# pimdh/lie-vae

Hardware: AMD Instinct MI355X
Metric: SO(3) samples/sec (exp+WignerD+action, l_max=10) (higher is better)
Workload: dtype f32

## Files before the change

### lie-vae_amd/csrc/action.hip

```cpp
#include <algorithm>
#include <cmath>
#include <cstdlib>
#include <array>
#include <atomic>
#include <vector>

#include "action_kernels.h"

namespace lv {
LV_EXTERN_LAUNCHERS(0) LV_EXTERN_LAUNCHERS(1) LV_EXTERN_LAUNCHERS(2) LV_EXTERN_LAUNCHERS(3)
LV_EXTERN_LAUNCHERS(4) LV_EXTERN_LAUNCHERS(5) LV_EXTERN_LAUNCHERS(6) LV_EXTERN_LAUNCHERS(7)
LV_EXTERN_LAUNCHERS(8) LV_EXTERN_LAUNCHERS(9) LV_EXTERN_LAUNCHERS(10) LV_EXTERN_LAUNCHERS(11)
LV_EXTERN_LAUNCHERS(12) LV_EXTERN_LAUNCHERS(13) LV_EXTERN_LAUNCHERS(14) LV_EXTERN_LAUNCHERS(15)
LV_EXTERN_LAUNCHERS(16) LV_EXTERN_LAUNCHERS(17) LV_EXTERN_LAUNCHERS(18) LV_EXTERN_LAUNCHERS(19)
LV_EXTERN_LAUNCHERS(20)
LV_EXTERN_BWD(0) LV_EXTERN_BWD(1) LV_EXTERN_BWD(2) LV_EXTERN_BWD(3) LV_EXTERN_BWD(4)
LV_EXTERN_BWD(5) LV_EXTERN_BWD(6) LV_EXTERN_BWD(7) LV_EXTERN_BWD(8) LV_EXTERN_BWD(9)
LV_EXTERN_BWD(10) LV_EXTERN_BWD(11) LV_EXTERN_BWD(12) LV_EXTERN_BWD(13) LV_EXTERN_BWD(14)
LV_EXTERN_BWD(15) LV_EXTERN_BWD(16) LV_EXTERN_BWD(17) LV_EXTERN_BWD(18) LV_EXTERN_BWD(19)
LV_EXTERN_BWD(20)

#ifndef LV_REDUCE_COLS
#define LV_REDUCE_COLS 16
#endif
constexpr int kBwdReduceCols = LV_REDUCE_COLS;
constexpr int kBwdReduceStreams = 64 / kBwdReduceCols;
__global__ __launch_bounds__(64 * kBwdReduceWaves) void action_bwd_reduce_kernel(
    const float* ws_F, float* gF, int64_t MC, int nslab) {
  __shared__ float part[kBwdReduceWaves][64];
  const int lane = threadIdx.x & 63, w = threadIdx.x >> 6;
  const int k = lane / kBwdReduceCols, col = lane - k * kBwdReduceCols;
  const int64_t e = (int64_t)blockIdx.x * kBwdReduceCols + col;
  const int per = (nslab + kBwdReduceWaves - 1) / kBwdReduceWaves;
  const int b0 = min(nslab, w * per), b1 = min(nslab, b0 + per);
  float sum = 0.f;
  if (e < MC) {
    int b = b0 + k;
    constexpr int S = kBwdReduceStreams;
    for (; b + 7 * S < b1; b += 8 * S) {
      float v[8];
#pragma unroll
      for (int u = 0; u < 8; ++u) v[u] = ws_F[(int64_t)(b + u * S) * MC + e];
#pragma unroll
      for (int u = 0; u < 8; ++u) sum += v[u];
    }
    for (; b < b1; b += S) sum += ws_F[(int64_t)b * MC + e];
  }
  part[w][lane] = sum;
  __syncthreads();
  if (threadIdx.x < kBwdReduceCols && e < MC) {
    float r = 0.f;
    for (int ww = 0; ww < kBwdReduceWaves; ++ww) {
      float rw = part[ww][col];
#pragma unroll
      for (int kk = 1; kk < kBwdReduceStreams; ++kk) rw += part[ww][kk * kBwdReduceCols + col];
      r += rw;
    }
    gF[e] = r;
  }
}

template <int COLS>
__global__ __launch_bounds__(1024) void action_bwd_reduce2_kernel(const float* ws_F, float* gF, int64_t MC,
                                                                  int nslab) {
  constexpr int S = 1024 / COLS;
  __shared__ float part[S][COLS];
  const int col = (int)threadIdx.x % COLS, k = (int)threadIdx.x / COLS;
  const int64_t e = (int64_t)blockIdx.x * COLS + col;
  float sum = 0.f;
  if (e < MC) {
    int b = k;
    for (; b + 7 * S < nslab; b += 8 * S) {
      float v[8];
#pragma unroll
      for (int u = 0; u < 8; ++u) v[u] = ws_F[(int64_t)(b + u * S) * MC + e];
#pragma unroll
      for (int u = 0; u < 8; ++u) sum += v[u];
    }
    for (; b < nslab; b += S) sum += ws_F[(int64_t)b * MC + e];
  }
  part[k][col] = sum;
#pragma unroll
  for (int h = S / 2; h >= 1; h >>= 1) {
    __syncthreads();
    if (k < h) part[k][col] += part[k + h][col];
  }
  if (k == 0 && e < MC) gF[e] = part[0][col];
}

__global__ __launch_bounds__(1024) void action_bwd_reduce3_kernel(const float* ws_F, float* gF, int64_t MC,
                                                                  int nslab, unsigned long long* stamps) {
  typedef float f4 __attribute__((ext_vector_type(4)));
  unsigned long long* rst = stamps ? stamps + kStampBlocks * 16 * 8 + 2 * (int64_t)blockIdx.x : nullptr;
  if (rst && threadIdx.x == 0) rst[0] = __builtin_amdgcn_s_memrealtime();
  __shared__ f4 part[256][4];
  const int q = (int)threadIdx.x & 3, bs = (int)threadIdx.x >> 2;
  const f4* base = reinterpret_cast<const f4*>(ws_F + (int64_t)blockIdx.x * nslab * kSlabChunk) + q;
  f4 acc = {0.f, 0.f, 0.f, 0.f};
  int b = bs;
  for (; b + 3 * 256 < nslab; b += 4 * 256) {
    f4 v[4];
#pragma unroll
    for (int u = 0; u < 4; ++u) v[u] = base[(int64_t)(b + u * 256) * 4];
#pragma unroll
    for (int u = 0; u < 4; ++u) acc += v[u];
  }
  {
    f4 v[3];
#pragma unroll
    for (int u = 0; u < 3; ++u) v[u] = b + u * 256 < nslab ? base[(int64_t)(b + u * 256) * 4] : f4{0.f, 0.f, 0.f, 0.f};
#pragma unroll
    for (int u = 0; u < 3; ++u)
      if (b + u * 256 < nslab) acc += v[u];
  }
  part[bs][q] = acc;
#pragma unroll
  for (int h = 128; h >= 1; h >>= 1) {
    __syncthreads();
    if (bs < h) part[bs][q] += part[bs + h][q];
  }
  if (bs == 0) {
    const f4 r = part[0][q];
#pragma unroll
    for (int k = 0; k < 4; ++k) {
      const int64_t e = (int64_t)blockIdx.x * kSlabChunk + 4 * q + k;
      if (e < MC) gF[e] = r[k];
    }
    if (rst) rst[1] = __builtin_amdgcn_s_memrealtime();
  }
}

__global__ __launch_bounds__(1024) void action_bwd_reduce4_kernel(const float* ws_F, float* gF, int64_t MC,
                                                                  int nslab) {
  typedef float f4 __attribute__((ext_vector_type(4)));
  __shared__ f4 part[16][4];
  const int q = (int)threadIdx.x & 3, bs = (int)threadIdx.x >> 2;
  const f4* base = reinterpret_cast<const f4*>(ws_F + (int64_t)blockIdx.x * nslab * kSlabChunk) + q;
  f4 acc = {0.f, 0.f, 0.f, 0.f};
  int b = bs;
  for (; b + 3 * 256 < nslab; b += 4 * 256) {
    f4 v[4];
#pragma unroll
    for (int u = 0; u < 4; ++u) v[u] = base[(int64_t)(b + u * 256) * 4];
#pragma unroll
    for (int u = 0; u < 4; ++u) acc += v[u];
  }
  {
    f4 v[3];
#pragma unroll
    for (int u = 0; u < 3; ++u) v[u] = b + u * 256 < nslab ? base[(int64_t)(b + u * 256) * 4] : f4{0.f, 0.f, 0.f, 0.f};
#pragma unroll
    for (int u = 0; u < 3; ++u)
      if (b + u * 256 < nslab) acc += v[u];
  }
#pragma unroll
  for (int m = 4; m <= 32; m <<= 1) {
#pragma unroll
    for (int k = 0; k < 4; ++k) acc[k] += __shfl_xor(acc[k], m, 64);
  }
  const int w = (int)threadIdx.x >> 6, lane = (int)threadIdx.x & 63;
  if (lane < 4) part[w][lane] = acc;
  __syncthreads();
  if (threadIdx.x < 4) {
    f4 r = part[0][q];
#pragma unroll
    for (int ww = 1; ww < 16; ++ww) r += part[ww][q];
#pragma unroll
    for (int k = 0; k < 4; ++k) {
      const int64_t e = (int64_t)blockIdx.x * kSlabChunk + 4 * q + k;
      if (e < MC) gF[e] = r[k];
    }
  }
}

constexpr int kR5Loads = 12;
__device__ __forceinline__ void reduce5_chunk(const float* ws_F, float* gF, int64_t MC, int nslab, int chunk) {
// ... 25 lines not shown
#pragma unroll
    for (int ww = 1; ww < 4; ++ww) r += part[ww][q];
#pragma unroll
    for (int k = 0; k < 4; ++k) {
      const int64_t e = (int64_t)chunk * kSlabChunk + 4 * q + k;
      if (e < MC) gF[e] = r[k];
    }
  }
}
__global__ __launch_bounds__(256) void action_bwd_reduce5_kernel(const float* ws_F, float* gF, int64_t MC, int nslab) {
  reduce5_chunk(ws_F, gF, MC, nslab, (int)blockIdx.x);
}

__global__ __launch_bounds__(256) void action_bwd_reduce5_vjp_kernel(const float* ws_F, float* gF, int64_t MC,
                                                                     int nslab, int nvjp, const float* mu,
                                                                     const float* v, const float* gang,
                                                                     float* gmu, float* gv, int64_t n) {
  if ((int)blockIdx.x < nvjp) {
    const int64_t i = (int64_t)blockIdx.x * 256 + threadIdx.x;
    if (i < n) {
      float av[3], g[3], m[9], gm[9], o[3];
#pragma unroll
      for (int k = 0; k < 3; ++k) { av[k] = v[i * 3 + k]; g[k] = gang[i * 3 + k]; }
      if (mu) {
#pragma unroll
        for (int k = 0; k < 9; ++k) m[k] = mu[i * 9 + k];
      }
      exp_eazyz_vjp_sample_wide(av, mu != nullptr, m, g, gm, o);
      if (mu) {
#pragma unroll
        for (int k = 0; k < 9; ++k) gmu[i * 9 + k] = gm[k];
      }
#pragma unroll
      for (int k = 0; k < 3; ++k) gv[i * 3 + k] = o[k];
    }
    return;
  }
  reduce5_chunk(ws_F, gF, MC, nslab, (int)blockIdx.x - nvjp);
}

namespace {

template <int... Ls>
constexpr std::array<int, sizeof...(Ls)> nnz_table(std::integer_sequence<int, Ls...>) {
  return {j_nnz<Ls>()...};
}
constexpr auto kNnz = nnz_table(std::make_integer_sequence<int, LV_MAX_DEGREE + 1>{});

inline double degree_cost(int l, bool bwd) {
  const int n = 2 * l + 1;
  const double fwd = 2.0 * kNnz[l] + 6.0 * n + 3.0 * n;
  return bwd ? 2.2 * fwd : fwd;
}

inline int plan_segments(int L, int nseg, double P, bool bwd, int* seg_lo) {
  constexpr int kD = LV_MAX_DEGREE + 1;
  const int D = L + 1;
  nseg = std::max(1, std::min(nseg, std::min(D, kMaxSeg)));
  double pre[kD + 1];
  pre[0] = 0.0;
  for (int l = 0; l < D; ++l) pre[l + 1] = pre[l] + degree_cost(l, bwd);
  const double INF = 1e30;
  double dp[kMaxSeg + 1][kD + 1];
  int arg[kMaxSeg + 1][kD + 1];
  for (int k = 0; k <= nseg; ++k)
    for (int i = 0; i <= D; ++i) { dp[k][i] = INF; arg[k][i] = 0; }
  dp[0][0] = 0.0;
  for (int k = 1; k <= nseg; ++k)
    for (int i = 1; i <= D; ++i)
      for (int p = k - 1; p < i; ++p) {
        const double v = std::max(dp[k - 1][p], pre[i] - pre[p] + P);
        if (v < dp[k][i]) { dp[k][i] = v; arg[k][i] = p; }
      }
  int i = D;
  for (int k = nseg; k >= 1; --k) {
    seg_lo[k] = i;
    i = arg[k][i];
  }
  seg_lo[0] = 0;
  return nseg;
}

constexpr double kDegFixedFwd = 80.0, kDegFixedBwd = 30.0;
inline double degree_cost_sched(int l, bool bwd) {
  return (bwd ? kDegFixedBwd : kDegFixedFwd) + degree_cost(l, bwd);
}
inline void balance_masks(int L, int nseg, bool bwd, unsigned* masks) {
  double load[kMaxSeg];
  for (int k = 0; k < nseg; ++k) { load[k] = 0.0; masks[k] = 0u; }
  for (int l = L; l >= 0; --l) {
    int best = 0;
    for (int k = 1; k < nseg; ++k)
      if (load[k] < load[best]) best = k;
    masks[best] |= 1u << l;
    load[best] += degree_cost_sched(l, bwd);
  }
  for (int k = nseg; k < kMaxSeg; ++k) masks[k] = 0u;
}
inline void contiguous_masks(const int* seg_lo, int nseg, unsigned* masks) {
  for (int k = 0; k < kMaxSeg; ++k) {
    masks[k] = 0u;
    if (k < nseg)
      for (int l = seg_lo[k]; l < seg_lo[k + 1]; ++l) masks[k] |= 1u << l;
  }
}

inline int choose_nseg(int64_t n, int Sw, int L, double P, bool bwd) {
  const int64_t waves = (n + Sw - 1) / Sw;
  const int64_t target = 2732;
  int nseg = (int)std::min<int64_t>(kMaxSeg, std::max<int64_t>(1, (target + waves - 1) / waves));
  double total = 0.0;
  for (int l = 0; l <= L; ++l) total += degree_cost(l, bwd);
  const int cap = std::max(1, (int)(total / (2.0 * P)));
  return std::min(nseg, std::min(cap, L + 1));
}

constexpr double kPrologueFwd = 200.0;
constexpr double kPrologueFused = 250.0;

constexpr size_t kTileMaxLds = 80 * 1024;
constexpr double kTileSegCostFew = 300.0;
constexpr double kTileSegCostMid = 260.0;
constexpr double kTileSegCostLarge = 560.0;
constexpr int64_t kTileFewGroupsPerCU = 4, kTileMidGroupsPerCU = 16;
constexpr double kTilePrologue = 60.0;
constexpr int64_t kWriteThroughMaxBytes = 32ll << 20;

#ifdef LV_AB_KNOBS
int env_int(const char* name, int dflt) {
  const char* v = std::getenv(name);
  return v && *v ? std::atoi(v) : dflt;
}
#define LV_KNOB(name, dflt) env_int(name, dflt)
constexpr size_t kStampBytes = sizeof(unsigned long long) * ((size_t)kStampDegBase + kStampDegBlocks * 16 * 24);
unsigned long long* ab_stamps() {
  static unsigned long long* p = nullptr;
  static bool tried = false;
  if (!tried) {
    tried = true;
    if (env_int("LV_STAMPS", 0) && hipMalloc(&p, kStampBytes) == hipSuccess) (void)hipMemset(p, 0, kStampBytes);
  }
  return p;
}
bool env_masks(const char* name, int L, int nseg, unsigned* masks) {
  const char* v = std::getenv(name);
  if (!v || !*v) return false;
  unsigned m[kMaxSeg] = {};
  int k = 0;
  unsigned all = 0;
  for (const char* s = v; *s && k < kMaxSeg;) {
    char* e = nullptr;
    m[k] = (unsigned)std::strtoul(s, &e, 16);
    if (e == s || (m[k] & all) || m[k] == 0) return false;
    all |= m[k++];
    s = (*e == ',' || *e == ':') ? e + 1 : e;
  }
  if (k != nseg || all != (1u << (L + 1)) - 1) return false;
  for (int i = 0; i < kMaxSeg; ++i) masks[i] = i < nseg ? m[i] : 0u;
  return true;
}
#else
#define LV_KNOB(name, dflt) (dflt)
inline unsigned long long* ab_stamps() { return nullptr; }
inline bool env_masks(const char*, int, int, unsigned*) { return false; }
#endif

int device_cus();

bool plan_tile(FwdLaunch& p, int L, int out_bytes, int cus) {
  static const int kEnvTile = LV_KNOB("LV_TILE", 1);
  static const int kEnvWT = LV_KNOB("LV_TILE_WT", -1);
  static const int kEnvTileNseg = LV_KNOB("LV_TILE_NSEG", 0);
  static const int kEnvPrio = LV_KNOB("LV_TILE_PRIO", 2);
  static const int kEnvSw = LV_KNOB("LV_TILE_SW", 0);
  if (!kEnvTile) return false;
  ActionArgs& a = p.a;
  int Sw = 64 / a.C;
  if (a.C == kTileFastC && kEnvSw >= 2 && kEnvSw < Sw) Sw = kEnvSw;
  const int64_t groups = (a.n + Sw - 1) / Sw;
  double total = 0.0;
  for (int l = 0; l <= L; ++l) total += degree_cost(l, false);
  const double target = groups <= kTileFewGroupsPerCU * cus   ? kTileSegCostFew
                        : groups <= kTileMidGroupsPerCU * cus ? kTileSegCostMid
                                                              : kTileSegCostLarge;
  int nseg = std::max(1, std::min(std::min(8, L + 1), (int)std::ceil(total / target)));
  if (kEnvTileNseg > 0) nseg = std::min(std::min(8, L + 1), kEnvTileNseg);
  nseg = std::min(L + 1, std::max(nseg, (3 * Sw + 63) / 64));
  if (3 * Sw > 64 * nseg || nseg > 8) return false;
  plan_segments(L, nseg, kTilePrologue, false, a.seg_lo);
  static const int kEnvContig = LV_KNOB("LV_SEG_CONTIG", 0);
  if (a.C == kTileFastC && env_masks("LV_TILE_MASKS", L, nseg, a.seg_mask)) {
  } else if (a.C == kTileFastC && !kEnvContig) balance_masks(L, nseg, false, a.seg_mask);
  else contiguous_masks(a.seg_lo, nseg, a.seg_mask);
  int fp = 0;
  if (a.C != kTileFastC && L < kTileFGlobalMinL)
    for (int k = 0; k < nseg; ++k) fp = std::max(fp, fseg_rows(a.seg_lo[k], a.seg_lo[k + 1]) * a.C);
  a.fpitch = (fp + 3) & ~3;
  const size_t fl = a.C == kTileFastC ? (out_bytes == 4 ? 0 : (size_t)a.MC) : (size_t)nseg * a.fpitch;
  const size_t trig = (size_t)Sw * (6 * ((L + 1 + 3) & ~3) + 4);
  const size_t lds = (size_t)tile_stage_bytes(Sw, a.MC, out_bytes) + sizeof(float) * (fl + trig);
  if (lds > kTileMaxLds || groups > 0x7fffffff) return false;
  a.Sw = Sw;
  a.write_through = (int64_t)a.n * a.MC * out_bytes <= kWriteThroughMaxBytes ? 1 : 0;
  if (kEnvWT >= 0) a.write_through = kEnvWT;
  a.prio = kEnvPrio;
  static const int kEnvSpread = LV_KNOB("LV_TILE_SPREAD", 0);
  a.task_spread = kEnvSpread;
  static const int kEnvAngOrder = LV_KNOB("LV_TILE_ANG_ORDER", 0);
  a.ang_order = kEnvAngOrder;
  p.tile = true;
  p.lds = lds;
  p.gx = (int)groups;
  p.gy = nseg;
  return true;
}

template <template <int> class Launcher, int LT = 0>
int dispatch_L(int L, typename Launcher<0>::Args& args) {
  if constexpr (LT > LV_MAX_DEGREE) {
    set_error("l_max %d > %d unsupported", L, LV_MAX_DEGREE);
    return LV_ERR_ARG;
  } else {
    if (L == LT) return Launcher<LT>::run(args);
    return dispatch_L<Launcher, LT + 1>(L, args);
  }
}

int check_common(int64_t n, int L, int C, int dtype) {
  LV_CHECK_ARG(n >= 0, "n must be >= 0 (got %lld)", (long long)n);
  LV_CHECK_ARG(L >= 0 && L <= LV_MAX_DEGREE, "l_max must be in [0, %d] (got %d)", LV_MAX_DEGREE, L);
  LV_CHECK_ARG(C >= 1 && C <= LV_MAX_CHANNELS, "C must be in [1, %d] (got %d)", LV_MAX_CHANNELS, C);
  LV_CHECK_ARG(dtype == LV_DTYPE_F32 || dtype == LV_DTYPE_BF16, "bad out dtype %d", dtype);
  return LV_OK;
}

int check_fwd(bool fused, int64_t Fstride, int out_dtype, int64_t n, int L, int C) {
  if (int e = check_common(n, L, C, out_dtype)) return e;
  const int64_t MC = (int64_t)(L + 1) * (L + 1) * C;
  LV_CHECK_ARG(Fstride == 0 || Fstride == MC, "F batch stride must be 0 or M*C=%lld", (long long)MC);
  LV_CHECK_ARG(!fused || Fstride == 0, "the fused path takes a shared spectrum (F batch stride 0)");
  LV_CHECK_ARG(Fstride == 0 || out_dtype == LV_DTYPE_F32, "bf16 output needs a shared spectrum");
  return LV_OK;
}

int plan_fwd(bool fused, int64_t Fstride, int out_dtype, int64_t n, int L, int C, int cus, FwdLaunch& p) {
  if (int e = check_fwd(fused, Fstride, out_dtype, n, L, C)) return e;
  const int64_t MC = (int64_t)(L + 1) * (L + 1) * C;
  p = FwdLaunch{};
  p.a.Fstride = Fstride;
  p.a.n = n;
  p.a.MC = MC;
  p.a.C = C;
  p.a.Sw = 64 / C;
  p.fused = fused;
  p.dtype = out_dtype;
  const int ob = out_dtype == LV_DTYPE_BF16 ? 2 : 4;
  if (Fstride == 0 && plan_tile(p, L, ob, cus)) return LV_OK;
  const double P = fused ? kPrologueFused : kPrologueFwd;
  static const int kEnvFwdNseg = LV_KNOB("LV_FWD_NSEG", 0);
  const int nseg = kEnvFwdNseg > 0 ? std::min(kEnvFwdNseg, std::min(L + 1, kMaxSeg))
                                   : choose_nseg(n, p.a.Sw, L, P, false);
  plan_segments(L, nseg, P, false, p.a.seg_lo);
  contiguous_masks(p.a.seg_lo, nseg, p.a.seg_mask);
  const int64_t gx = (n + (int64_t)p.a.Sw * kWavesPerBlock - 1) / ((int64_t)p.a.Sw * kWavesPerBlock);
  LV_CHECK_ARG(gx <= 0x7fffffff, "batch too large");
  p.gx = (int)gx;
  p.gy = nseg;
  int fmax = 0;
  if (Fstride == 0)
    for (int k = 0; k < nseg; ++k)
      fmax = std::max(fmax, (fseg_rows(p.a.seg_lo[k], p.a.seg_lo[k + 1]) * C + 3) & ~3);
  p.a.fpitch = fmax;
  const size_t trig = L >= kTrigLdsMinL ? (size_t)kWavesPerBlock * p.a.Sw * trig_row_floats(L) : 0;
  p.lds = sizeof(float) * ((size_t)fmax + trig);
  return LV_OK;
}

template <class K, class V, int N = 8>
struct PlanCache {
  K key[N];
  V val[N];
  int used = 0, next = 0;
  const V* find(const K& k) const {
    for (int i = 0; i < used; ++i)
      if (key[i] == k) return &val[i];
    return nullptr;
  }
  void put(const K& k, const V& v) {
    key[next] = k;
    val[next] = v;
    next = (next + 1) % N;
// ... 432 lines not shown
```

### lie-vae_amd/csrc/action_common.h

```cpp
#pragma once
#include "action_chain.h"
#include "so3_device.h"

namespace lv {

constexpr int kWavesPerBlock = 4;
constexpr int kThreads = 64 * kWavesPerBlock;
constexpr int kMaxSeg = 16;
constexpr int kTrigLdsMinL = 13;
constexpr int kTileFGlobalMinL = 13;

struct ActionArgs {
  const float* ang;
  const float* mu;
  const float* v;
  const float* F;
  int64_t Fstride;
  void* out;
  float* ang_out;
  int64_t n;
  int64_t MC;
  int C, Sw, transpose;
  int fpitch;
  int write_through;
  int prio;
  int task_spread;
  int ang_order;
  unsigned long long* stamps;
  int seg_lo[kMaxSeg + 1];
  unsigned seg_mask[kMaxSeg];
};

constexpr int64_t kStampBlocks = 16384;
__device__ __forceinline__ void phase_stamp(unsigned long long* st, int wave, int k) {
  if (st && (threadIdx.x & 63) == 0 && blockIdx.x < kStampBlocks)
    st[((int64_t)blockIdx.x * 16 + wave) * 8 + k] = __builtin_amdgcn_s_memrealtime();
}
constexpr int64_t kStampDegBlocks = 2048;
constexpr int64_t kStampDegBase = kStampBlocks * 16 * 8 + 2 * 4096;
__device__ __forceinline__ void degree_stamp(unsigned long long* st, int wave, int l) {
  if (st && (threadIdx.x & 63) == 0 && blockIdx.x < kStampDegBlocks)
    st[kStampDegBase + ((int64_t)blockIdx.x * 16 + wave) * 24 + l] = __builtin_amdgcn_s_memrealtime();
}



__device__ __forceinline__ void quat_to_zyz_trig(const float q[4], float c1[3], float s1[3]) {
  const float a1 = q[1] * q[2] - q[0] * q[3];
  const float b1 = q[0] * q[2] + q[1] * q[3];
  const float cb = ((q[3] * q[3] - q[0] * q[0]) - q[1] * q[1]) + q[2] * q[2];
  const float a3 = q[0] * q[3] + q[1] * q[2];
  const float b3 = q[1] * q[3] - q[0] * q[2];
  auto dir = [](float y, float x, float& c, float& s) {
    const float r2 = x * x + y * y;
    if (r2 == 0.f) {
      c = signbit(x) ? -1.f : 1.f;
      s = 0.f;
    } else {
      const float r = rsqrtf(r2);
      c = x * r;
      s = y * r;
    }
  };
  dir(a1, b1, c1[0], s1[0]);
  const float x = fminf(fmaxf(cb, kEazyzLo), kEazyzHi);
  c1[1] = x;
  s1[1] = sqrtf((1.f - x) * (1.f + x));
  dir(a3, b3, c1[2], s1[2]);
}

__device__ __forceinline__ void lv_sincos(float x, float& s, float& c) {
  const float k = rintf(x * 0.63661977236758134f);
  float r = fmaf(k, -1.5707963705062866f, x);
  r = fmaf(k, 4.371138828673793e-08f, r);
  r = fmaf(k, 1.7151245100058819e-15f, r);
  const float r2 = r * r;
  const float ps = fmaf(r2, fmaf(r2, -1.9515295891e-4f, 8.3321608736e-3f), -1.6666654611e-1f) * r2;
  const float sn = fmaf(r, ps, r);
  const float pc = fmaf(r2, fmaf(r2, 2.443315711809948e-5f, -1.388731625493765e-3f), 4.166664568298827e-2f);
  const float cs = fmaf(r2 * r2, pc, fmaf(r2, -0.5f, 1.f));
  const int q = (int)k & 3;
  s = (q & 1) ? cs : sn;
  c = (q & 1) ? sn : cs;
  if (q == 1 || q == 2) c = -c;
  if (q >= 2) s = -s;
  if (__builtin_expect(!(fabsf(x) <= 1.0e5f), 0)) sincosf(x, &s, &c);
}

struct ExpQuat {
  float qr[4];
  float qk2, rd;
};
__device__ __forceinline__ ExpQuat exp_quat(const float v[3]) {
  ExpQuat e;
  const float vv = v[0] * v[0] + v[1] * v[1] + v[2] * v[2];
  const float inv = rsqrtf(vv);
  const float th = vv * inv;
  float sh, ch;
  lv_sincos(0.5f * th, sh, ch);
  const float m = -sh * inv;
  const float qt[4] = {v[0] * m, v[1] * m, v[2] * m, ch};
  int k = 0;
  float best = fabsf(qt[0]);
#pragma unroll
  for (int i = 1; i < 4; ++i)
    if (fabsf(qt[i]) > best) { best = fabsf(qt[i]); k = i; }
  const float qk = k == 0 ? qt[0] : (k == 1 ? qt[1] : (k == 2 ? qt[2] : qt[3]));
  constexpr float eps = 2.5e-7f;
  e.qk2 = qk * qk;
  e.rd = rsqrtf(e.qk2 + eps);
  const float d = (e.qk2 + eps) * e.rd;
  const float sc = copysignf(best * e.rd, qk);
#pragma unroll
  for (int i = 0; i < 4; ++i) e.qr[i] = (i == k) ? d : qt[i] * sc;
  return e;
}
__device__ __forceinline__ void exp_beta(const ExpQuat& e, float& c, float& s) {
  constexpr float eps = 2.5e-7f;
  const float* qr = e.qr;
  const float oms = eps * (1.f - 2.f * e.qk2 - eps) * (e.rd * e.rd);
  float omc = fmaf(2.f, qr[0] * qr[0] + qr[1] * qr[1], oms);
  float opc = fmaf(2.f, qr[2] * qr[2] + qr[3] * qr[3], oms);
  constexpr float kDelta = 1.f - kEazyzHi;
  const bool clo = omc < kDelta, chi = !clo && opc < kDelta;
  omc = clo ? kDelta : (chi ? 2.f - kDelta : omc);
// ... 156 lines not shown
```

### lie-vae_amd/csrc/action_fwd.h

```cpp
#pragma once
#include <type_traits>
#include "action_common.h"

namespace lv {

template <int LT, bool FUSED, bool SHARED, typename OutT>
__global__ __launch_bounds__(kThreads) void action_fwd_kernel(ActionArgs a) {
  extern __shared__ float lds[];
  const int lane = threadIdx.x & 63;
  const int wave = __builtin_amdgcn_readfirstlane(threadIdx.x >> 6);
  const int C = a.C, Sw = a.Sw;
  const int j = lane / C;
  const int c = lane - j * C;
  const int lo = a.seg_lo[blockIdx.y], hi = a.seg_lo[blockIdx.y + 1];
  const int rows_lo = lo * lo;
  const int frows = SHARED ? fseg_rows(lo, hi) : 0;
  const int64_t s0 = ((int64_t)blockIdx.x * kWavesPerBlock + wave) * Sw;
  const int Sv = (int)max((int64_t)0, min((int64_t)Sw, a.n - s0));
  const bool active = j < Sv;
  const int64_t s = active ? s0 + j : (Sv > 0 ? s0 : 0);
  LaneIn in;
  if (Sv > 0) lane_load<FUSED>(a, s, in);
  constexpr int kFPer = 8;
  float fv[kFPer];
// ... 89 lines not shown
          const float v1 = odd ? y[i + 1] : recv;
          if (active) store_out2(d, v0, v1);
          d += 2 * C;
        });
        if (active) store_out(out + s * a.MC + (r0 + nn - 1) * C + c, y[nn - 1]);
      } else if (active) {
        OutT* d = out + s * a.MC + r0 * C + c;
        sfor<nn>([&](auto I) {
          store_out(d, y[LV_CV(I)]);
          d += C;
        });
      }
    }
  });
}

typedef float lv_f4 __attribute__((ext_vector_type(4)));

template <int POL>
__device__ __forceinline__ void tile_store16(__amdgpu_buffer_rsrc_t r, int off, lv_f4 v) {
  __builtin_amdgcn_raw_buffer_store_b128(v, r, off, 0, POL);
}
template <int POL>
__device__ __forceinline__ void tile_store_elem(__amdgpu_buffer_rsrc_t r, int off, float v) {
  __builtin_amdgcn_raw_buffer_store_b32(__builtin_bit_cast(unsigned int, v), r, off, 0, POL);
}
template <int POL>
__device__ __forceinline__ void tile_store_elem(__amdgpu_buffer_rsrc_t r, int off,
                                                __hip_bfloat16 v) {
  __builtin_amdgcn_raw_buffer_store_b16(__builtin_bit_cast(short, v), r, off, 0, POL);
}
__device__ __forceinline__ float tile_cvt(float v, float*) { return v; }
__device__ __forceinline__ __hip_bfloat16 tile_cvt(float v, __hip_bfloat16*) {
  return __float2bfloat16(v);
}

constexpr int kRawBufferFlags = 0x00020000;

__host__ __device__ inline int tile_stage_bytes(int Sw, int64_t MC, int out_bytes) {
  return (int)((((int64_t)Sw * MC * out_bytes + 16) + 15) & ~(int64_t)15);
}

template <typename OutT, int POL>
__device__ __forceinline__ void tile_flush(OutT* gout, const char* stage_b, int mis, int nbytes,
                                           int tid, int nthr) {
  const int head = min((16 - mis) & 15, nbytes);
  const int nvec = (nbytes - head) >> 4;
  const int tail0 = head + nvec * 16;
  const __amdgpu_buffer_rsrc_t rs =
      __builtin_amdgcn_make_buffer_rsrc(gout, 0, nbytes, kRawBufferFlags);
  for (int k = tid; k < nvec; k += nthr) {
    const lv_f4 v = *reinterpret_cast<const lv_f4*>(stage_b + head + 16 * k);
    tile_store16<POL>(rs, head + 16 * k, v);
  }
  constexpr int E = (int)sizeof(OutT);
  const int nedge = head / E + (nbytes - tail0) / E;
  if (tid < nedge) {
    const int b = tid < head / E ? tid * E : tail0 + (tid - head / E) * E;
    tile_store_elem<POL>(rs, b, *reinterpret_cast<const OutT*>(stage_b + b));
  }
}

__device__ __forceinline__ void block_sync_lds() {
  asm volatile("s_waitcnt lgkmcnt(0)\n\ts_barrier" ::: "memory");
}

template <typename OutT>
__device__ __forceinline__ void tile_flush_rt(OutT* gout, const char* stage_b, int mis, int nbytes,
                                              int write_through) {
  if (write_through == 1)
    tile_flush<OutT, 16>(gout, stage_b, mis, nbytes, (int)threadIdx.x, (int)blockDim.x);
  else if (write_through == 2)
    tile_flush<OutT, 0>(gout, stage_b, mis, nbytes, (int)threadIdx.x, (int)blockDim.x);
  else
    tile_flush<OutT, 1>(gout, stage_b, mis, nbytes, (int)threadIdx.x, (int)blockDim.x);
}

template <int LT, int CT, bool FUSED, typename OutT, bool MAYMU = true>
__device__ __forceinline__ void fwd_tile_body(const ActionArgs& a, int64_t grp) {
  extern __shared__ __attribute__((aligned(16))) float lds[];
  constexpr int kRow = TrigLds<LT>::kRow;
  constexpr bool FG = CT == 0 && LT >= kTileFGlobalMinL;
  constexpr bool FT = CT > 0 && std::is_same_v<OutT, float>;
  const int C = CT > 0 ? CT : a.C;
  const int Sw = a.Sw;
  const int64_t MC = CT > 0 ? (int64_t)(LT + 1) * (LT + 1) * CT : a.MC;
  const int lane = threadIdx.x & 63;
  const int wave = __builtin_amdgcn_readfirstlane(threadIdx.x >> 6);
  const int tid = (int)threadIdx.x, nthr = (int)blockDim.x;
  const int j = lane / C;
  const int c = lane - j * C;
  const unsigned dmask = a.seg_mask[wave];
  const int lo = a.seg_lo[wave], hi = a.seg_lo[wave + 1];
  const int rows_lo = lo * lo;
  const int frows = fseg_rows(lo, hi);
  const int64_t s0 = grp * Sw;
  const int Sv = (int)min((int64_t)Sw, a.n - s0);
  const bool active = j < Sv;
  const int stage_bytes = tile_stage_bytes(Sw, MC, (int)sizeof(OutT));
  float* trig = lds + (stage_bytes >> 2);
  OutT* gout = reinterpret_cast<OutT*>(a.out) + s0 * MC;
  const int mis = (int)(reinterpret_cast<uintptr_t>(gout) & 15);
  char* stage_b = reinterpret_cast<char*>(lds) + mis;
  float* const Fall = FT ? reinterpret_cast<float*>(stage_b) + (Sw - 1) * MC : trig + Sw * kRow;
  float* Fw = Fall + (CT > 0 ? 0 : wave * a.fpitch);
  phase_stamp(a.stamps, wave, 0);
  if (a.prio >= 2) __builtin_amdgcn_s_setprio(3);
  const int t_task = a.task_spread ? lane * (nthr >> 6) + wave : tid;
  const bool task = t_task < 3 * Sw;
  const int jt = t_task / 3, q = t_task - 3 * (t_task / 3);
  const int64_t st = s0 + min(jt, Sv - 1);
  LaneIn in;
  if (task) lane_load<FUSED, MAYMU>(a, st, in);
  constexpr bool kAngLate = FUSED && !MAYMU;
  const int ang_wave = (nthr >> 6) > 1 ? 1 : 0;
  const int beta_wave = (nthr >> 6) > 2 ? 2 : ang_wave;
  const bool ang_on = kAngLate && a.ang_out != nullptr && lane < Sv;
  const bool ang_lane = ang_on && wave == ang_wave;
  const bool beta_lane = ang_on && wave == beta_wave;
  auto write_ang = [&](bool dirs, bool beta) {
    float vang[3];
#pragma unroll
    for (int i = 0; i < 3; ++i) vang[i] = a.v[(s0 + lane) * 3 + i];
    const ExpQuat e = exp_quat(vang);
    if (dirs) {
      float ang[3];
      quat_to_eazyz_fwd(e.qr, ang);
      a.ang_out[(s0 + lane) * 3 + 0] = ang[0];
      a.ang_out[(s0 + lane) * 3 + 2] = ang[2];
    }
    if (beta) {
      float cb, sb;
      exp_beta(e, cb, sb);
      a.ang_out[(s0 + lane) * 3 + 1] = saved_beta(cb, sb);
    }
  };
  const bool early_dirs = ang_lane && ang_wave == 1, early_beta = beta_lane && beta_wave >= 1;
  if ((early_dirs || early_beta) && a.ang_order == 0) write_ang(early_dirs, early_beta);
  constexpr int kFPer = FG ? 1 : (CT > 0 ? ((LT + 1) * (LT + 1) * (CT > 0 ? CT : 1) + 127) / 128 : 6);
  constexpr int kFPerCap = kFPer < 18 ? kFPer : 18;
  float fv[kFPerCap];
  const int fcnt = FG ? 0 : (CT > 0 ? (int)MC : (hi * hi - rows_lo) * C);
  const int fstr = CT > 0 ? nthr : 64;
  const int fbase = CT > 0 ? tid : lane;
  const float* fsrc = a.F + (CT > 0 ? 0 : rows_lo * C);
#pragma unroll
  for (int k = 0; k < kFPerCap; ++k) {
    const int e = fbase + fstr * k;
    fv[k] = e < fcnt ? fsrc[e] : 0.f;
  }
  if ((early_dirs || early_beta) && a.ang_order != 0) write_ang(early_dirs, early_beta);
  if (a.stamps) {
    asm volatile("s_waitcnt vmcnt(0)" ::: "memory");
    phase_stamp(a.stamps, wave, 5);
  }
  if (task) {
    float cq, sq;
    if constexpr (FUSED && !MAYMU) {
      float qr[4];
      exp_to_zyz_slot(in.v, a.transpose ? 2 - q : q, cq, sq, qr);
      if (a.transpose) sq = -sq;
    } else {
      float c1[3], s1[3];
      lane_angles<FUSED, MAYMU>(a, in, st, jt < Sv, q, FUSED && a.ang_out != nullptr, c1, s1);
      cq = q == 0 ? c1[0] : (q == 1 ? c1[1] : c1[2]);
      sq = q == 0 ? s1[0] : (q == 1 ? s1[1] : s1[2]);
    }
    if (a.stamps) phase_stamp(a.stamps, wave, 6);
    trig_row_fill1<LT>(trig + jt * kRow, cq, sq, q, LT);
    if (a.stamps) phase_stamp(a.stamps, wave, 7);
  }
  if constexpr (FG) {
  } else if constexpr (CT > 0) {
#pragma unroll
    for (int k = 0; k < kFPerCap; ++k) {
      const int e = fbase + fstr * k;
      if (e < fcnt) Fw[e] = fv[k];
    }
    for (int e0 = fbase + fstr * kFPerCap; e0 < fcnt; e0 += 8 * fstr) {
      float t8[8];
#pragma unroll
      for (int u = 0; u < 8; ++u) t8[u] = e0 + fstr * u < fcnt ? fsrc[e0 + fstr * u] : 0.f;
#pragma unroll
      for (int u = 0; u < 8; ++u)
        if (e0 + fstr * u < fcnt) Fw[e0 + fstr * u] = t8[u];
    }
  } else {
#pragma unroll
    for (int k = 0; k < kFPerCap; ++k) {
      const int e = lane + 64 * k;
      if (e < fcnt) {
        const int r = e / C, cc = e - r * C;
        Fw[cc * frows + r] = fv[k];
      }
    }
    for (int e = lane + 64 * kFPerCap; e < fcnt; e += 64) {
      const int r = e / C, cc = e - r * C;
      Fw[cc * frows + r] = fsrc[e];
    }
  }
  block_sync_lds();
  phase_stamp(a.stamps, wave, 1);

  if (a.prio >= 2) __builtin_amdgcn_s_setprio(0);
  OutT* st_lane = reinterpret_cast<OutT*>(stage_b) + j * MC + c;
  const float* tj = trig + min(j, Sw - 1) * kRow;
  const float* Fl = FG ? a.F + c : (CT > 0 ? Fall + c : Fw + c * frows - rows_lo);
  const int fstep = (FG || CT > 0) ? C : 1;

  sfor<LT + 1>([&](auto Lc) {
    constexpr int l = LV_CV(Lc);
    if ((dmask >> l) & 1u) {
      constexpr int nn = 2 * l + 1;
      constexpr int r0 = l * l;
      float x[nn], y[nn];
      sfor<nn>([&](auto K) { x[LV_CV(K)] = Fl[(r0 + LV_CV(K)) * fstep]; });
      xrot_lds<l, 2, LT>(tj, x, y);
      jmul<l>(y, x);
      xrot_lds<l, 1, LT>(tj, x, y);
      jmul<l>(y, x);
      xrot_lds<l, 0, LT>(tj, x, y);
      if (active) {
        OutT* d = st_lane + r0 * C;
        sfor<nn>([&](auto I) {
          d[0] = tile_cvt(y[LV_CV(I)], (OutT*)nullptr);
          d += C;
        });
      }
      if (a.stamps) degree_stamp(a.stamps, wave, l);
    }
  });
  if (ang_lane && ang_wave == 0) write_ang(true, true);
  phase_stamp(a.stamps, wave, 2);
  block_sync_lds();
  phase_stamp(a.stamps, wave, 3);
  if (a.prio == 1) __builtin_amdgcn_s_setprio(3);
  else if (a.prio == 3) __builtin_amdgcn_s_setprio(2);
  tile_flush_rt<OutT>(gout, stage_b, mis, Sv * (int)MC * (int)sizeof(OutT), a.write_through);
  phase_stamp(a.stamps, wave, 4);
}

template <int LT, int CT, bool FUSED, typename OutT, bool MAYMU = true>
__global__ __launch_bounds__(512) void action_fwd_tile_kernel(ActionArgs a) {
  fwd_tile_body<LT, CT, FUSED, OutT, MAYMU>(a, blockIdx.x);
}


template <int l>
__global__ void wigner_d_kernel(const float* ang, float* D, int64_t n, int dsz) {
  constexpr int nn = 2 * l + 1;
  const int64_t tid = (int64_t)blockIdx.x * blockDim.x + threadIdx.x;
  if (tid >= n * nn) return;
  const int64_t s = tid / nn;
  const int q = (int)(tid - s * nn);
  float c1[3], s1[3];
  for (int i = 0; i < 3; ++i) sincosf(ang[s * 3 + i], &s1[i], &c1[i]);
  TrigTab<l> t;
  trig_fill<l>(t, c1, s1, l);
  float x[nn], y[nn];
  sfor<nn>([&](auto K) { x[LV_CV(K)] = (LV_CV(K) == q) ? 1.f : 0.f; });
  xrot<l, 2>(t, x, y);
  jmul<l>(y, x);
  xrot<l, 1>(t, x, y);
  jmul<l>(y, x);
  xrot<l, 0>(t, x, y);
  constexpr int off = l * (2 * l - 1) * (2 * l + 1) / 3;
  sfor<nn>([&](auto I) { D[s * dsz + off + LV_CV(I) * nn + q] = y[LV_CV(I)]; });
}


constexpr int kTileFastC = 10;

struct FwdLaunch {
  ActionArgs a;
  int gx, gy;
  bool fused;
  bool tile;
  size_t lds;
  int dtype;
  hipStream_t stream;
};

template <int LT>
struct FwdLauncher {
  using Args = FwdLaunch;
  template <int CT>
  static void launch_tile(FwdLaunch& p, bool bf16);
  static int run(FwdLaunch& p);
};

template <int LT>
template <int CT>
void FwdLauncher<LT>::launch_tile(FwdLaunch& p, bool bf16) {
  const dim3 grid(p.gx), block(64 * p.gy);
  if (p.fused && CT > 0 && !p.a.mu) {
    if (bf16)
      hipLaunchKernelGGL((action_fwd_tile_kernel<LT, CT, true, __hip_bfloat16, false>), grid, block, p.lds, p.stream, p.a);
    else
      hipLaunchKernelGGL((action_fwd_tile_kernel<LT, CT, true, float, false>), grid, block, p.lds, p.stream, p.a);
  } else if (p.fused) {
    if (bf16)
      hipLaunchKernelGGL((action_fwd_tile_kernel<LT, CT, true, __hip_bfloat16>), grid, block, p.lds, p.stream, p.a);
    else
      hipLaunchKernelGGL((action_fwd_tile_kernel<LT, CT, true, float>), grid, block, p.lds, p.stream, p.a);
  } else {
    if (bf16)
      hipLaunchKernelGGL((action_fwd_tile_kernel<LT, CT, false, __hip_bfloat16>), grid, block, p.lds, p.stream, p.a);
    else
      hipLaunchKernelGGL((action_fwd_tile_kernel<LT, CT, false, float>), grid, block, p.lds, p.stream, p.a);
  }
}

template <int LT>
int FwdLauncher<LT>::run(FwdLaunch& p) {
  const bool bf16 = p.dtype == LV_DTYPE_BF16;
  if (p.tile) {
    if (p.a.C == kTileFastC)
      launch_tile<kTileFastC>(p, bf16);
    else
      launch_tile<0>(p, bf16);
    LV_RETURN_LAUNCH("action_fwd_tile_kernel");
// ... 50 lines not shown
```

Measured before the change: 594.2 million.

## Streamline tile kernel prologue: compile out stamps, reorder args, buffer loads

```diff
diff --git a/lie-vae_amd/csrc/action.hip b/lie-vae_amd/csrc/action.hip
--- a/lie-vae_amd/csrc/action.hip
+++ b/lie-vae_amd/csrc/action.hip
@@ -91,7 +91,7 @@
 __global__ __launch_bounds__(1024) void action_bwd_reduce3_kernel(const float* ws_F, float* gF, int64_t MC,
                                                                   int nslab, unsigned long long* stamps) {
   typedef float f4 __attribute__((ext_vector_type(4)));
-  unsigned long long* rst = stamps ? stamps + kStampBlocks * 16 * 8 + 2 * (int64_t)blockIdx.x : nullptr;
+  unsigned long long* rst = kStamps && stamps ? stamps + kStampBlocks * 16 * 8 + 2 * (int64_t)blockIdx.x : nullptr;
   if (rst && threadIdx.x == 0) rst[0] = __builtin_amdgcn_s_memrealtime();
   __shared__ f4 part[256][4];
   const int q = (int)threadIdx.x & 3, bs = (int)threadIdx.x >> 2;
@@ -283,16 +283,21 @@
 }
 
 constexpr double kDegFixedFwd = 80.0, kDegFixedBwd = 30.0;
+constexpr double kAngChargeDirs = 220.0, kAngChargeBeta = 150.0;
 inline double degree_cost_sched(int l, bool bwd) {
   return (bwd ? kDegFixedBwd : kDegFixedFwd) + degree_cost(l, bwd);
 }
-inline void balance_masks(int L, int nseg, bool bwd, unsigned* masks) {
+inline void balance_masks(int L, int nseg, bool bwd, unsigned* masks, const double* charge = nullptr) {
   double load[kMaxSeg];
-  for (int k = 0; k < nseg; ++k) { load[k] = 0.0; masks[k] = 0u; }
+  for (int k = 0; k < nseg; ++k) { load[k] = charge ? charge[k] : 0.0; masks[k] = 0u; }
+  int empty = nseg;
   for (int l = L; l >= 0; --l) {
-    int best = 0;
-    for (int k = 1; k < nseg; ++k)
-      if (load[k] < load[best]) best = k;
+    int best = -1;
+    for (int k = 0; k < nseg; ++k) {
+      if (l + 1 <= empty && masks[k] != 0u) continue;
+      if (best < 0 || load[k] < load[best]) best = k;
+    }
+    if (masks[best] == 0u) --empty;
     masks[best] |= 1u << l;
     load[best] += degree_cost_sched(l, bwd);
   }
@@ -390,9 +395,16 @@
   if (3 * Sw > 64 * nseg || nseg > 8) return false;
   plan_segments(L, nseg, kTilePrologue, false, a.seg_lo);
   static const int kEnvContig = LV_KNOB("LV_SEG_CONTIG", 0);
+  static const int kEnvAngOrder = LV_KNOB("LV_TILE_ANG_ORDER", 0);
   if (a.C == kTileFastC && env_masks("LV_TILE_MASKS", L, nseg, a.seg_mask)) {
-  } else if (a.C == kTileFastC && !kEnvContig) balance_masks(L, nseg, false, a.seg_mask);
-  else contiguous_masks(a.seg_lo, nseg, a.seg_mask);
+  } else if (a.C == kTileFastC && !kEnvContig) {
+    double charge[kMaxSeg] = {};
+    if (p.fused && kEnvAngOrder != 0 && nseg > 1) {
+      charge[1] = nseg > 2 ? kAngChargeDirs : kAngChargeDirs + kAngChargeBeta;
+      if (nseg > 2) charge[2] = kAngChargeBeta;
+    }
+    balance_masks(L, nseg, false, a.seg_mask, charge);
+  } else contiguous_masks(a.seg_lo, nseg, a.seg_mask);
   int fp = 0;
   if (a.C != kTileFastC && L < kTileFGlobalMinL)
     for (int k = 0; k < nseg; ++k) fp = std::max(fp, fseg_rows(a.seg_lo[k], a.seg_lo[k + 1]) * a.C);
@@ -407,7 +419,6 @@
   a.prio = kEnvPrio;
   static const int kEnvSpread = LV_KNOB("LV_TILE_SPREAD", 0);
   a.task_spread = kEnvSpread;
-  static const int kEnvAngOrder = LV_KNOB("LV_TILE_ANG_ORDER", 0);
   a.ang_order = kEnvAngOrder;
   p.tile = true;
   p.lds = lds;
diff --git a/lie-vae_amd/csrc/action_common.h b/lie-vae_amd/csrc/action_common.h
--- a/lie-vae_amd/csrc/action_common.h
+++ b/lie-vae_amd/csrc/action_common.h
@@ -1,6 +1,7 @@
 #pragma once
 #include "action_chain.h"
 #include "so3_device.h"
+#include <cstddef>
 
 namespace lv {
 
@@ -10,37 +11,50 @@
 constexpr int kTrigLdsMinL = 13;
 constexpr int kTileFGlobalMinL = 13;
 
-struct ActionArgs {
-  const float* ang;
-  const float* mu;
+struct alignas(64) ActionArgs {
   const float* v;
   const float* F;
-  int64_t Fstride;
   void* out;
   float* ang_out;
   int64_t n;
-  int64_t MC;
-  int C, Sw, transpose;
-  int fpitch;
-  int write_through;
+  int Sw;
   int prio;
   int task_spread;
+  int transpose;
   int ang_order;
+  int write_through;
+  unsigned seg_mask[kMaxSeg];
+  const float* ang;
+  const float* mu;
+  int64_t Fstride;
+  int64_t MC;
+  int C;
+  int fpitch;
   unsigned long long* stamps;
   int seg_lo[kMaxSeg + 1];
-  unsigned seg_mask[kMaxSeg];
 };
-
+static_assert(offsetof(ActionArgs, seg_mask) == 64 && offsetof(ActionArgs, ang) == 128,
+              "ActionArgs: the tile kernel's start-up fields fill the first two 64-byte lines");
+
+#ifdef LV_AB_KNOBS
+constexpr bool kStamps = true;
+#else
+constexpr bool kStamps = false;
+#endif
 constexpr int64_t kStampBlocks = 16384;
 __device__ __forceinline__ void phase_stamp(unsigned long long* st, int wave, int k) {
-  if (st && (threadIdx.x & 63) == 0 && blockIdx.x < kStampBlocks)
-    st[((int64_t)blockIdx.x * 16 + wave) * 8 + k] = __builtin_amdgcn_s_memrealtime();
+  if constexpr (kStamps) {
+    if (st && (threadIdx.x & 63) == 0 && blockIdx.x < kStampBlocks)
+      st[((int64_t)blockIdx.x * 16 + wave) * 8 + k] = __builtin_amdgcn_s_memrealtime();
+  }
 }
 constexpr int64_t kStampDegBlocks = 2048;
 constexpr int64_t kStampDegBase = kStampBlocks * 16 * 8 + 2 * 4096;
 __device__ __forceinline__ void degree_stamp(unsigned long long* st, int wave, int l) {
-  if (st && (threadIdx.x & 63) == 0 && blockIdx.x < kStampDegBlocks)
-    st[kStampDegBase + ((int64_t)blockIdx.x * 16 + wave) * 24 + l] = __builtin_amdgcn_s_memrealtime();
+  if constexpr (kStamps) {
+    if (st && (threadIdx.x & 63) == 0 && blockIdx.x < kStampDegBlocks)
+      st[kStampDegBase + ((int64_t)blockIdx.x * 16 + wave) * 24 + l] = __builtin_amdgcn_s_memrealtime();
+  }
 }
 
 
diff --git a/lie-vae_amd/csrc/action_fwd.h b/lie-vae_amd/csrc/action_fwd.h
--- a/lie-vae_amd/csrc/action_fwd.h
+++ b/lie-vae_amd/csrc/action_fwd.h
@@ -195,108 +195,150 @@
   constexpr int kRow = TrigLds<LT>::kRow;
   constexpr bool FG = CT == 0 && LT >= kTileFGlobalMinL;
   constexpr bool FT = CT > 0 && std::is_same_v<OutT, float>;
-  const int C = CT > 0 ? CT : a.C;
-  const int Sw = a.Sw;
-  const int64_t MC = CT > 0 ? (int64_t)(LT + 1) * (LT + 1) * CT : a.MC;
   const int lane = threadIdx.x & 63;
   const int wave = __builtin_amdgcn_readfirstlane(threadIdx.x >> 6);
-  const int tid = (int)threadIdx.x, nthr = (int)blockDim.x;
+  const int tid = (int)threadIdx.x;
+  const float* const vin = FUSED ? a.v : a.ang;
+  const float* const aF = a.F;
+  void* const aout = a.out;
+  float* const aang = a.ang_out;
+  const int64_t an = a.n;
+  const int Sw = a.Sw;
+  const int prio = a.prio, spread = a.task_spread, transp = a.transpose;
+  const int ang_order = a.ang_order, wthrough = a.write_through;
+  const unsigned dmask = a.seg_mask[wave];
+  const int nthr = (int)blockDim.x;
+  asm volatile("" ::"s"(vin), "s"(aF), "s"(aout), "s"(aang), "s"(an), "s"(Sw), "s"(prio), "s"(spread),
+               "s"(transp), "s"(ang_order), "s"(wthrough), "s"(dmask), "s"(nthr));
+  phase_stamp(a.stamps, wave, 0);
+  if (prio >= 2) __builtin_amdgcn_s_setprio(3);
+  const int nw = nthr >> 6;
+  const int64_t s0 = grp * Sw;
+  const int Sv = (int)min((int64_t)Sw, an - s0);
+  const __amdgpu_buffer_rsrc_t vrs = __builtin_amdgcn_make_buffer_rsrc(
+      const_cast<float*>(vin) + s0 * 3, 0, Sv * 12, kRawBufferFlags);
+  auto load3 = [&](int js, float x[3]) {
+#pragma unroll
+    for (int i = 0; i < 3; ++i)
+      x[i] = __builtin_bit_cast(float, __builtin_amdgcn_raw_buffer_load_b32(vrs, js * 12 + 4 * i, 0, 0));
+  };
+  const int t_task = spread ? lane * nw + wave : tid;
+  const bool task = t_task < 3 * Sw;
+  const int jt = (t_task * 683) >> 11, q = t_task - 3 * jt;
+  const int64_t st = s0 + min(jt, Sv - 1);
+  LaneIn in;
+  if (task) {
+    load3(min(jt, Sv - 1), in.v);
+    if constexpr (FUSED && MAYMU) {
+      if (a.mu) {
+#pragma unroll
+        for (int i = 0; i < 9; ++i) in.mu[i] = a.mu[st * 9 + i];
+      }
+    }
+  }
+  const int C = CT > 0 ? CT : a.C;
+  const int64_t MC = CT > 0 ? (int64_t)(LT + 1) * (LT + 1) * CT : a.MC;
   const int j = lane / C;
   const int c = lane - j * C;
-  const unsigned dmask = a.seg_mask[wave];
   const int lo = a.seg_lo[wave], hi = a.seg_lo[wave + 1];
   const int rows_lo = lo * lo;
   const int frows = fseg_rows(lo, hi);
-  const int64_t s0 = grp * Sw;
-  const int Sv = (int)min((int64_t)Sw, a.n - s0);
   const bool active = j < Sv;
   const int stage_bytes = tile_stage_bytes(Sw, MC, (int)sizeof(OutT));
   float* trig = lds + (stage_bytes >> 2);
-  OutT* gout = reinterpret_cast<OutT*>(a.out) + s0 * MC;
+  OutT* gout = reinterpret_cast<OutT*>(aout) + s0 * MC;
   const int mis = (int)(reinterpret_cast<uintptr_t>(gout) & 15);
   char* stage_b = reinterpret_cast<char*>(lds) + mis;
   float* const Fall = FT ? reinterpret_cast<float*>(stage_b) + (Sw - 1) * MC : trig + Sw * kRow;
   float* Fw = Fall + (CT > 0 ? 0 : wave * a.fpitch);
-  phase_stamp(a.stamps, wave, 0);
-  if (a.prio >= 2) __builtin_amdgcn_s_setprio(3);
-  const int t_task = a.task_spread ? lane * (nthr >> 6) + wave : tid;
-  const bool task = t_task < 3 * Sw;
-  const int jt = t_task / 3, q = t_task - 3 * (t_task / 3);
-  const int64_t st = s0 + min(jt, Sv - 1);
-  LaneIn in;
-  if (task) lane_load<FUSED, MAYMU>(a, st, in);
   constexpr bool kAngLate = FUSED && !MAYMU;
-  const int ang_wave = (nthr >> 6) > 1 ? 1 : 0;
-  const int beta_wave = (nthr >> 6) > 2 ? 2 : ang_wave;
-  const bool ang_on = kAngLate && a.ang_out != nullptr && lane < Sv;
-  const bool ang_lane = ang_on && wave == ang_wave;
-  const bool beta_lane = ang_on && wave == beta_wave;
-  auto write_ang = [&](bool dirs, bool beta) {
-    float vang[3];
-#pragma unroll
-    for (int i = 0; i < 3; ++i) vang[i] = a.v[(s0 + lane) * 3 + i];
+  const int ang_wave = nw > 1 ? 1 : 0;
+  const int beta_wave = nw > 2 ? 2 : ang_wave;
+  const bool ang_on = kAngLate && aang != nullptr && lane < Sv;
+  const bool dirs_lane = ang_on && wave == ang_wave, beta_lane = ang_on && wave == beta_wave;
+  const bool ang_early = ang_order == 0 && nw > 1;
+  float vang[3] = {0.f, 0.f, 0.f};
+  if (dirs_lane || beta_lane) load3(lane, vang);
+  auto write_ang = [&]() {
+    const __amdgpu_buffer_rsrc_t ars =
+        __builtin_amdgcn_make_buffer_rsrc(aang + s0 * 3, 0, Sv * 12, kRawBufferFlags);
     const ExpQuat e = exp_quat(vang);
-    if (dirs) {
+    if (dirs_lane) {
       float ang[3];
       quat_to_eazyz_fwd(e.qr, ang);
-      a.ang_out[(s0 + lane) * 3 + 0] = ang[0];
-      a.ang_out[(s0 + lane) * 3 + 2] = ang[2];
-    }
-    if (beta) {
+      __builtin_amdgcn_raw_buffer_store_b32(__builtin_bit_cast(unsigned int, ang[0]), ars, lane * 12, 0, 0);
+      __builtin_amdgcn_raw_buffer_store_b32(__builtin_bit_cast(unsigned int, ang[2]), ars, lane * 12 + 8, 0, 0);
+    }
+    if (beta_lane) {
       float cb, sb;
       exp_beta(e, cb, sb);
-      a.ang_out[(s0 + lane) * 3 + 1] = saved_beta(cb, sb);
+      __builtin_amdgcn_raw_buffer_store_b32(__builtin_bit_cast(unsigned int, saved_beta(cb, sb)), ars,
+                                            lane * 12 + 4, 0, 0);
     }
   };
-  const bool early_dirs = ang_lane && ang_wave == 1, early_beta = beta_lane && beta_wave >= 1;
-  if ((early_dirs || early_beta) && a.ang_order == 0) write_ang(early_dirs, early_beta);
+  if constexpr (kAngLate) {
+    if ((dirs_lane || beta_lane) && ang_early) write_ang();
+  }
   constexpr int kFPer = FG ? 1 : (CT > 0 ? ((LT + 1) * (LT + 1) * (CT > 0 ? CT : 1) + 127) / 128 : 6);
   constexpr int kFPerCap = kFPer < 18 ? kFPer : 18;
+  constexpr int kMCT = (LT + 1) * (LT + 1) * (CT > 0 ? CT : 1);
+  constexpr int kSlots7 = (kMCT + 447) / 448 < kFPerCap ? (kMCT + 447) / 448 : kFPerCap;
+  constexpr int kSlots4 = (kMCT + 255) / 256 < kFPerCap ? (kMCT + 255) / 256 : kFPerCap;
+  static_assert(CT == 0 || kSlots4 * 256 >= kMCT, "tile staging: the 4-wave tier covers the spectrum");
   float fv[kFPerCap];
   const int fcnt = FG ? 0 : (CT > 0 ? (int)MC : (hi * hi - rows_lo) * C);
   const int fstr = CT > 0 ? nthr : 64;
   const int fbase = CT > 0 ? tid : lane;
-  const float* fsrc = a.F + (CT > 0 ? 0 : rows_lo * C);
-#pragma unroll
-  for (int k = 0; k < kFPerCap; ++k) {
-    const int e = fbase + fstr * k;
-    fv[k] = e < fcnt ? fsrc[e] : 0.f;
-  }
-  if ((early_dirs || early_beta) && a.ang_order != 0) write_ang(early_dirs, early_beta);
-  if (a.stamps) {
-    asm volatile("s_waitcnt vmcnt(0)" ::: "memory");
-    phase_stamp(a.stamps, wave, 5);
+  const float* fsrc = aF + (CT > 0 ? 0 : rows_lo * C);
+  if constexpr (CT > 0) {
+    auto ld = [&](auto K) { fv[LV_CV(K)] = fsrc[min(tid + nthr * LV_CV(K), kMCT - 1)]; };
+    if (nw >= 7) sfor<kSlots7>(ld);
+    else if (nw >= 4) sfor<kSlots4>(ld);
+    else sfor<kFPerCap>(ld);
+  } else {
+#pragma unroll
+    for (int k = 0; k < kFPerCap; ++k) {
+      const int e = fbase + fstr * k;
+      fv[k] = e < fcnt ? fsrc[e] : 0.f;
+    }
+  }
+  if constexpr (kStamps) {
+    if (a.stamps) {
+      asm volatile("s_waitcnt vmcnt(0)" ::: "memory");
+      phase_stamp(a.stamps, wave, 5);
+    }
   }
   if (task) {
     float cq, sq;
     if constexpr (FUSED && !MAYMU) {
       float qr[4];
-      exp_to_zyz_slot(in.v, a.transpose ? 2 - q : q, cq, sq, qr);
-      if (a.transpose) sq = -sq;
+      exp_to_zyz_slot(in.v, transp ? 2 - q : q, cq, sq, qr);
+      if (transp) sq = -sq;
     } else {
       float c1[3], s1[3];
-      lane_angles<FUSED, MAYMU>(a, in, st, jt < Sv, q, FUSED && a.ang_out != nullptr, c1, s1);
+      lane_angles<FUSED, MAYMU>(a, in, st, jt < Sv, q, FUSED && aang != nullptr, c1, s1);
       cq = q == 0 ? c1[0] : (q == 1 ? c1[1] : c1[2]);
       sq = q == 0 ? s1[0] : (q == 1 ? s1[1] : s1[2]);
     }
-    if (a.stamps) phase_stamp(a.stamps, wave, 6);
+    phase_stamp(a.stamps, wave, 6);
     trig_row_fill1<LT>(trig + jt * kRow, cq, sq, q, LT);
-    if (a.stamps) phase_stamp(a.stamps, wave, 7);
+    phase_stamp(a.stamps, wave, 7);
   }
   if constexpr (FG) {
   } else if constexpr (CT > 0) {
-#pragma unroll
-    for (int k = 0; k < kFPerCap; ++k) {
-      const int e = fbase + fstr * k;
-      if (e < fcnt) Fw[e] = fv[k];
-    }
-    for (int e0 = fbase + fstr * kFPerCap; e0 < fcnt; e0 += 8 * fstr) {
-      float t8[8];
-#pragma unroll
-      for (int u = 0; u < 8; ++u) t8[u] = e0 + fstr * u < fcnt ? fsrc[e0 + fstr * u] : 0.f;
-#pragma unroll
-      for (int u = 0; u < 8; ++u)
-        if (e0 + fstr * u < fcnt) Fw[e0 + fstr * u] = t8[u];
+    auto wr = [&](auto K) { Fw[min(tid + nthr * LV_CV(K), kMCT - 1)] = fv[LV_CV(K)]; };
+    if (nw >= 7) sfor<kSlots7>(wr);
+    else if (nw >= 4) sfor<kSlots4>(wr);
+    else {
+      sfor<kFPerCap>(wr);
+      for (int e0 = fbase + fstr * kFPerCap; e0 < fcnt; e0 += 8 * fstr) {
+        float t8[8];
+#pragma unroll
+        for (int u = 0; u < 8; ++u) t8[u] = e0 + fstr * u < fcnt ? fsrc[e0 + fstr * u] : 0.f;
+#pragma unroll
+        for (int u = 0; u < 8; ++u)
+          if (e0 + fstr * u < fcnt) Fw[e0 + fstr * u] = t8[u];
+      }
     }
   } else {
 #pragma unroll
@@ -315,10 +357,13 @@
   block_sync_lds();
   phase_stamp(a.stamps, wave, 1);
 
-  if (a.prio >= 2) __builtin_amdgcn_s_setprio(0);
+  if (prio >= 2) __builtin_amdgcn_s_setprio(0);
+  if constexpr (kAngLate) {
+    if ((dirs_lane || beta_lane) && !ang_early) write_ang();
+  }
   OutT* st_lane = reinterpret_cast<OutT*>(stage_b) + j * MC + c;
   const float* tj = trig + min(j, Sw - 1) * kRow;
-  const float* Fl = FG ? a.F + c : (CT > 0 ? Fall + c : Fw + c * frows - rows_lo);
+  const float* Fl = FG ? aF + c : (CT > 0 ? Fall + c : Fw + c * frows - rows_lo);
   const int fstep = (FG || CT > 0) ? C : 1;
 
   sfor<LT + 1>([&](auto Lc) {
@@ -340,16 +385,15 @@
           d += C;
         });
       }
-      if (a.stamps) degree_stamp(a.stamps, wave, l);
+      degree_stamp(a.stamps, wave, l);
     }
   });
-  if (ang_lane && ang_wave == 0) write_ang(true, true);
   phase_stamp(a.stamps, wave, 2);
   block_sync_lds();
   phase_stamp(a.stamps, wave, 3);
-  if (a.prio == 1) __builtin_amdgcn_s_setprio(3);
-  else if (a.prio == 3) __builtin_amdgcn_s_setprio(2);
-  tile_flush_rt<OutT>(gout, stage_b, mis, Sv * (int)MC * (int)sizeof(OutT), a.write_through);
+  if (prio == 1) __builtin_amdgcn_s_setprio(3);
+  else if (prio == 3) __builtin_amdgcn_s_setprio(2);
+  tile_flush_rt<OutT>(gout, stage_b, mis, Sv * (int)MC * (int)sizeof(OutT), wthrough);
   phase_stamp(a.stamps, wave, 4);
 }
 
```

Result: faster. 625.6 million, median of 6 (+5.3%).
